# suleka96/siddhi

Hardware: AMD Instinct MI355X
Metric: input events/sec + % HBM peak, partitioned pattern query, 1/2/4/8 MI355X (higher is better)
Workload: dtype f64

## Files before the change

### siddhi_amd/csrc/kernels/stack_dev.h

```cpp
#pragma once
#include "fastpath_dev.h"

namespace sm {
namespace {

constexpr int kKeys = 1024;
#ifndef SM_STACK_KC
#define SM_STACK_KC 5
#endif
constexpr int kC = SM_STACK_KC;
constexpr int kQ = 32;
constexpr int kOB = 1024;
#ifndef SM_ORDER_TB
#define SM_ORDER_TB 13
#endif
constexpr int kTB = SM_ORDER_TB;
constexpr int kOT = 1 << kTB;

enum : uint32_t { SE_OVERFLOW = 1, SE_LOG = 2, SE_NAN = 4, SE_CAND = 8, SE_ORD = 16 };

struct ExactSrc {
  bool exact_codes;
  int vtype, vattr, cwidth;
  const void* vcol;
  const int64_t* ord;
  int64_t obase, n;
  const int64_t* crow;
  int32_t o0;
  uint32_t cs, ce;
  __device__ bool carried(uint32_t o) const { return (int32_t)o < o0; }
  __device__ int64_t row_of(uint32_t o) const {
    if (!ord) return o;
    const int64_t want = (int64_t)o + obase;
    int64_t lo = 0, hi = n - 1;
    while (lo < hi) {
      const int64_t mid = (lo + hi) >> 1;
      if (ord[mid] < want) lo = mid + 1;
      else hi = mid;
    }
    return lo;
  }
  __device__ int64_t carry_row(uint32_t o) const {
    const int64_t want = (int64_t)(int32_t)o + obase;
    uint32_t lo = cs, hi = ce;
    while (lo + 1 < hi) {
      const uint32_t mid = (lo + hi) >> 1;
      if (crow[(int64_t)mid * cwidth + 1] <= want) lo = mid;
      else hi = mid;
    }
    return lo;
  }
  __device__ double fval(uint32_t o) const {
    if (carried(o)) return __longlong_as_double((long long)crow[carry_row(o) * cwidth + 3 + vattr]);
    const int64_t r = row_of(o);
    return vtype == T_FLOAT ? (double)((const float*)vcol)[r] : ((const double*)vcol)[r];
  }
  __device__ int64_t ival(uint32_t o) const {
    if (carried(o)) return crow[carry_row(o) * cwidth + 3 + vattr];
    const int64_t r = row_of(o);
    return vtype == T_INT ? (int64_t)((const int32_t*)vcol)[r] : ((const int64_t*)vcol)[r];
  }
};

#ifndef SM_EXACT_INLINE
#define SM_EXACT_INLINE __noinline__
#endif
template <int OP, bool FP>
__device__ SM_EXACT_INLINE bool c2_exact_v(bool exact_codes, int vtype, int vattr, int cwidth, const void* vcol,
                                        const int64_t* ord, int64_t obase, int64_t n, const int64_t* crow, int32_t o0,
                                        uint32_t cs, uint32_t ce, uint32_t oi, uint32_t oj) {
  const ExactSrc ex{exact_codes, vtype, vattr, cwidth, vcol, ord, obase, n, crow, o0, cs, ce};
  if constexpr (FP) return cmp_fixed<OP>(ex.fval(oj), ex.fval(oi));
  else return cmp_fixed<OP>(ex.ival(oj), ex.ival(oi));
}
template <int OP, bool FP>
__device__ __forceinline__ bool c2_exact(const ExactSrc& ex, uint32_t oi, uint32_t oj) {
  return c2_exact_v<OP, FP>(ex.exact_codes, ex.vtype, ex.vattr, ex.cwidth, ex.vcol, ex.ord, ex.obase, ex.n, ex.crow,
                            ex.o0, ex.cs, ex.ce, oi, oj);
}

template <int OP, bool FP>
__device__ __forceinline__ bool c2_hit(const ExactSrc& ex, uint32_t ci, uint32_t oi, uint32_t cj, uint32_t oj) {
  const bool nan = FP & ((ci == kNanCode) | (cj == kNanCode));
  if (!nan & (ex.exact_codes | (ci != cj))) return cmp_fixed<OP>(cj, ci);
  return c2_exact<OP, FP>(ex, oi, oj);
}

struct Stack {
  uint32_t o[kC], c[kC];
  int32_t t[kC];
  int n;
  int hb, hn;
};

__device__ __forceinline__ void st_pop(Stack& s) {
#pragma unroll
  for (int k = 0; k + 1 < kC; ++k) {
    s.o[k] = s.o[k + 1];
    s.c[k] = s.c[k + 1];
    s.t[k] = s.t[k + 1];
  }
  --s.n;
}

__device__ __forceinline__ void st_refill(Stack& s, const uint4* sp) {
  const uint4 e = sp[(s.hb + s.hn - 1) & (kQ - 1)];
  s.o[0] = e.x;
  s.c[0] = e.y;
  s.t[0] = (int32_t)e.z;
  s.hn -= 1;
  s.n = 1;
}

__device__ __forceinline__ void st_push(Stack& s, uint4* sp, uint32_t o, uint32_t c, int32_t t, int32_t now,
                                        int64_t within, uint32_t* err) {
  if (s.n == kC) {
    if (within >= 0 && now - s.t[kC - 1] > (int32_t)within) {
      s.hn = 0;
      s.n = kC - 1;
    } else {
      if (s.hn == kQ) {
#pragma unroll 1
        while (s.hn > 0 && within >= 0 && now - (int32_t)sp[s.hb & (kQ - 1)].z > (int32_t)within) {
          s.hb = (s.hb + 1) & (kQ - 1);
          --s.hn;
        }
        if (s.hn == kQ) {
          atomicOr(err, SE_OVERFLOW);
          s.hb = (s.hb + 1) & (kQ - 1);
          --s.hn;
        }
      }
      sp[(s.hb + s.hn) & (kQ - 1)] = make_uint4(s.o[kC - 1], s.c[kC - 1], (uint32_t)s.t[kC - 1], 0u);
      ++s.hn;
      s.n = kC - 1;
    }
  }
#pragma unroll
  for (int k = kC - 1; k > 0; --k) {
    s.o[k] = s.o[k - 1];
    s.c[k] = s.c[k - 1];
    s.t[k] = s.t[k - 1];
  }
  s.o[0] = o;
  s.c[0] = c;
  s.t[0] = t;
  ++s.n;
}

template <int NT = kOB>
__device__ __forceinline__ uint32_t block_excl(uint32_t v, uint32_t* lw, uint32_t* tot) {
  const int lane = threadIdx.x & 63, w = threadIdx.x >> 6;
  uint32_t inc = v;
#pragma unroll
  for (int o = 1; o < 64; o <<= 1) {
    const uint32_t u = __shfl_up(inc, o, 64);
    if (lane >= o) inc += u;
  }
  if (lane == 63) lw[w] = inc;
  lds_barrier();
  uint32_t r = inc - v, t = 0;
  for (int q = 0; q < NT / 64; ++q) {
    const uint32_t x = lw[q];
    if (q < w) r += x;
    t += x;
  }
  *tot = t;
  return r;
}

#ifndef SM_STACK_R
#define SM_STACK_R 2
#endif
#ifndef SM_STACK_SS
#define SM_STACK_SS 3072
#endif
constexpr int kR = SM_STACK_R;
constexpr int kSS = SM_STACK_SS;
constexpr int kT4 = kKeys;
constexpr int kW4 = kT4 / 64;
constexpr int kI4 = kSS / kT4;
constexpr int kPool = kSS / 2;
static_assert(kSS % kT4 == 0 && kI4 * 64 <= 255 && kW4 == 16, "u8 per-(key, wave) counts, 16 waves");
static_assert(kSS <= 32768, "arrival positions | c1 fit 16 bits");

struct Slot4 {
  uint2 grp[kSS];
  uint32_t ordt[kSS];
  uint32_t pk[kSS];
  uint2 pool[kPool];
  uint32_t kst[kKeys];
  uint16_t epos[kSS];
  uint8_t jc[kSS];
};
static_assert(sizeof(uint32_t) * kSS + sizeof(uint2) * kPool >= kKeys * kW4, "ranking counts fit pk + pool");

struct Stack4Cold {
  int64_t kmin, ts0, within, obase, n;
  int vtype, vattr, cwidth;
  int32_t o0;
  bool exact_codes;
  const void* vcol;
  const int64_t* ord;
  const uint4* cin;
  const uint32_t* cstart;
  const uint32_t* cend;
  const int64_t* crow;
  int64_t* cand;
  uint32_t* cand_n;
  uint32_t cand_cap;
};

#ifndef SM_EXACT4_INLINE
#define SM_EXACT4_INLINE __noinline__
#endif
struct Stack4Args {
  const uint4* rec;
  const uint32_t* dbase;
  uint32_t n;
  int H;
  int32_t within;
  bool exact_codes;
  uint32_t ntiles;
  const uint32_t* sbase;
  uint64_t* stage;
  uint32_t* mstart;
  uint32_t* mtot;
  uint4* spill;
  uint32_t* err;
  const Stack4Cold* cold;
  unsigned long long* stamps;
};

#ifndef SM_STACK4_SKIP
#define SM_STACK4_SKIP 0
#endif
#ifndef SM_STACK4_STAMPS
#define SM_STACK4_STAMPS 0
#endif
#if SM_STACK4_STAMPS && defined(__HIP_DEVICE_COMPILE__)
#define SM4_CLOCK() __builtin_amdgcn_s_memtime()
#else
#define SM4_CLOCK() 0ull
#endif
#define SM4_PHASE(i)                              \
  do {                                            \
    if (SM_STACK4_STAMPS) {                       \
      const unsigned long long t_ = SM4_CLOCK();  \
      st_acc[i] += t_ - st_last;                  \
      st_last = t_;                               \
    }                                             \
  } while (0)

template <int OP, bool FP>
__device__ SM_EXACT4_INLINE bool c2_exact4(const Stack4Cold* c, uint32_t cs, uint32_t ce, uint32_t oi, uint32_t oj) {
  return c2_exact_v<OP, FP>(c->exact_codes, c->vtype, c->vattr, c->cwidth, c->vcol, c->ord, c->obase, c->n, c->crow,
                            c->o0, cs, ce, oi, oj);
}

__device__ __forceinline__ uint32_t sm4_opaque(uint32_t v) {
#if defined(__HIP_DEVICE_COMPILE__)
  asm volatile("" : "+v"(v));
#endif
  return v;
}

__device__ __forceinline__ void sm4_arrived(uint4 (&pre)[kI4]) {
#if defined(__HIP_DEVICE_COMPILE__)
#pragma unroll
  for (int k = 0; k < kI4; ++k)
    asm volatile("" : "+v"(pre[k].x), "+v"(pre[k].y), "+v"(pre[k].z), "+v"(pre[k].w) : : "memory");
#else
  (void)pre;
#endif
}

#ifndef SM_RANK4_INLINE
#define SM_RANK4_INLINE __forceinline__
#endif
__device__ SM_RANK4_INLINE void rank4(Slot4& S, const uint4 (&pre)[kI4], int sn, uint32_t* lw, bool fp,
                                       uint32_t* err) {
  const int tid = threadIdx.x, lane = tid & 63, w = wave_index();
  uint8_t* cnt = (uint8_t*)S.pk;
  {
    const uint32_t z = sm4_opaque(0u);
    *(uint4*)(cnt + 16 * tid) = make_uint4(z, z, z, z);
  }
  lds_barrier();
  uint32_t hk[kI4], lp[kI4];
  bool nan = false;
#pragma unroll
  for (int k = 0; k < kI4; ++k) {
    const int e = w * 64 * kI4 + k * 64 + lane;
    const bool valid = e < sn;
    nan |= fp && valid && pre[k].z == kNanCode;
    hk[k] = valid ? (pre[k].x & kKeyMask) >> kRB : 0u;
    const uint64_t peers = peer_mask(hk[k], valid);
    uint32_t old = 0;
    if (valid) old = cnt[16 * hk[k] + w];
    wave_lockstep();
    const uint32_t below = lanes_below(peers);
    if (valid && below == 0) cnt[16 * hk[k] + w] = (uint8_t)(old + (uint32_t)__popcll(peers));
    wave_lockstep();
    lp[k] = old + below;
  }
  if (__any(nan) && lane == 0) atomicOr(err, SE_NAN);
  lds_barrier();
  {
    const uint4 c = *(const uint4*)(cnt + 16 * tid);
    const uint32_t ones = 0x01010101u;
    const uint32_t tot = sm_udot4(c.x, ones, 0u) + sm_udot4(c.y, ones, 0u) +
                         sm_udot4(c.z, ones, 0u) + sm_udot4(c.w, ones, 0u);
    uint32_t all;
    const uint32_t st = block_excl<kT4>(tot, lw, &all);
    S.kst[tid] = st | (tot << 16);
  }
  lds_barrier();
#pragma unroll
  for (int k = 0; k < kI4; ++k) {
    const int e = w * 64 * kI4 + k * 64 + lane;
    if (e < sn) {
      const uint4 c = *(const uint4*)(cnt + 16 * hk[k]);
      const uint32_t wb = (uint32_t)w * 8u;
      auto part = [&](uint32_t word, uint32_t lo) {
        const uint32_t nb = wb > lo ? (wb - lo >= 32u ? 32u : wb - lo) : 0u;
        const uint32_t m = nb >= 32u ? 0xffffffffu : ((1u << nb) - 1u);
        return sm_udot4(word & m, 0x01010101u, 0u);
      };
      const uint32_t before = part(c.x, 0) + part(c.y, 32) + part(c.z, 64) + part(c.w, 96);
      const uint32_t pos = (S.kst[hk[k]] & 0xffffu) + before + lp[k];
      S.grp[pos] = make_uint2(pre[k].z, pre[k].w);
      S.epos[pos] = (uint16_t)((uint32_t)e | ((pre[k].x >> 31) << 15));
      S.ordt[e] = pre[k].y;
      if (SM_STACK4_SKIP) S.jc[e] = 0;
    }
  }
  lds_barrier();
}

template <int OP, bool FP>
__global__ void __launch_bounds__(kT4) stack4_kernel(Stack4Args a) {
  __shared__ __attribute__((aligned(16))) Slot4 sl[kR];
  __shared__ uint32_t lw[kW4];
  __shared__ uint32_t s_pool[kR];
  __shared__ uint32_t s_lastj, s_tot;
  const int tid = threadIdx.x, lane = tid & 63;
  const int h = tid;
  const bool has = h < a.H;
  const int32_t within32 = a.within;
  uint4* sp = a.spill + ((int64_t)blockIdx.x * kKeys + h) * kQ;
  unsigned long long st_acc[5] = {0, 0, 0, 0, 0}, st_last = SM4_CLOCK();

  for (int d = blockIdx.x; d < kBins; d += gridDim.x) {
    const uint32_t b0 = a.dbase[d];
    const uint32_t blen = (d + 1 < kBins ? a.dbase[d + 1] : a.n) - b0;
    const uint32_t nsl = (blen + kSS - 1) / kSS;
    const uint4* recb = a.rec + b0;
    uint64_t* stb = a.stage + a.sbase[d];
    uint32_t* mst = a.mstart + (int64_t)d * (a.ntiles + 1);
    const uint32_t kr = ((uint32_t)h << kRB) | (uint32_t)d;
    Stack st;
    st.n = st.hb = st.hn = 0;
    uint32_t cs = 0, ce = 0;
    if (has && a.cold->cin) {
      const Stack4Cold* c4 = a.cold;
      cs = c4->cstart[kr];
      ce = c4->cend[kr];
      for (uint32_t q = cs; q < ce; ++q) {
        const uint4 c = c4->cin[q];
        st_push(st, sp, c.x, c.y, (int32_t)c.z, (int32_t)c.z, within32, a.err);
      }
    }
    int32_t tl = 0;
    bool seen = false;
    uint32_t mrun = 0;
    __syncthreads();
    if (tid == 0) s_lastj = 0xffffffffu;
    if (tid < kR) s_pool[tid] = 0;

    uint4 pre[kI4];
    auto load = [&](uint32_t s) {
#pragma unroll
      for (int k = 0; k < kI4; ++k) {
        const uint32_t p = s * kSS + (uint32_t)wave_index() * 64 * kI4 + k * 64 + lane;
        if (p < blen) {
          typedef unsigned int u32x4 __attribute__((ext_vector_type(4)));
          const u32x4 v = __builtin_nontemporal_load((const u32x4*)recb + p);
          pre[k] = make_uint4(v.x, v.y, v.z, v.w);
        }
      }
    };
    auto slice_n = [&](uint32_t s) { return (int)(blen - s * kSS < (uint32_t)kSS ? blen - s * kSS : (uint32_t)kSS); };
    uint32_t off[kR], cnt[kR];
    SM4_PHASE(4);
    for (uint32_t s = 0; s < (uint32_t)kR; ++s) {
      off[s] = cnt[s] = 0;
      if (s < nsl) {
        load(s);
        rank4(sl[s], pre, slice_n(s), lw, FP, a.err);
        const uint32_t v = sl[s].kst[h];
        off[s] = v & 0xffffu;
        cnt[s] = v >> 16;
      }
    }
    if (kR < nsl) load(kR);

    SM4_PHASE(0);
    for (uint32_t e = 0; e < nsl; ++e) {
      const int q0 = (int)(e % kR);
      while (!SM_STACK4_SKIP && __any(cnt[0] != 0)) {
        int k = kR - 1;
#pragma unroll
        for (int u = kR - 2; u >= 0; --u)
          if (cnt[u]) k = u;
        uint32_t o_ = off[kR - 1], c_ = cnt[kR - 1];
#pragma unroll
        for (int u = kR - 2; u >= 0; --u)
          if (u == k) {
            o_ = off[u];
            c_ = cnt[u];
          }
        if (c_ != 0) {
#pragma unroll
        for (int u = 0; u < kR; ++u)
          if (u == k) {
            off[u] = o_ + 1;
            cnt[u] = c_ - 1;
          }
        const int q = q0 + k >= kR ? q0 + k - kR : q0 + k;
        Slot4& S = sl[q];
        const uint2 g = S.grp[o_];
        const uint32_t ep = S.epos[o_];
        const uint32_t p = ep & 0x7fffu;
        const uint32_t cj = g.x;
        const int32_t jt = (int32_t)g.y;
        tl = jt;
        seen = true;
        uint32_t hit = 0, exp = 0, tie = 0;
#pragma unroll
        for (int u = 0; u < kC; ++u) {
          const bool lv = u < st.n;
          hit |= (lv && cmp_fixed<OP>(cj, st.c[u])) ? (1u << u) : 0u;
          exp |= (lv && within32 >= 0 && jt - st.t[u] > within32) ? (1u << u) : 0u;
          tie |= (lv && !a.exact_codes && st.c[u] == cj) ? (1u << u) : 0u;
        }
        if (tie) {
          const uint32_t oj = S.ordt[p];
#pragma unroll 1
          for (uint32_t m = tie; m; m &= m - 1u) {
            const int u = __builtin_ctz(m);
            uint32_t oi = st.o[0];
#pragma unroll
            for (int v = 1; v < kC; ++v)
              if (v == u) oi = st.o[v];
            if (c2_exact4<OP, FP>(a.cold, cs, ce, oi, oj)) hit |= 1u << u;
            else hit &= ~(1u << u);
          }
        }
        const uint32_t ok = hit & ~exp;
        uint32_t npop = (uint32_t)__builtin_ctz(~ok);
        if (npop > (uint32_t)st.n) npop = st.n;
        const bool stop_expired = npop < (uint32_t)st.n && ((exp >> npop) & 1u);
        const bool cont = !stop_expired && npop == (uint32_t)st.n && st.hn > 0;
        if (npop) S.pk[p] = st.o[0];
        if (npop > 1) {
          const uint32_t base = atomicAdd(&s_pool[q], npop - 1u);
          if (base + npop - 1u > (uint32_t)kPool) atomicOr(a.err, SE_LOG);
#pragma unroll
          for (int u = 1; u < kC; ++u)
            if ((uint32_t)u < npop && base + u - 1u < (uint32_t)kPool)
              S.pool[base + u - 1u] = make_uint2(st.o[u], p | ((uint32_t)u << 16));
        }
#pragma unroll
        for (int b = 1; b < kC; b <<= 1)
          if (npop & b) {
#pragma unroll
            for (int u = 0; u < kC; ++u)
              if (u + b < kC) {
                st.o[u] = st.o[u + b];
                st.c[u] = st.c[u + b];
                st.t[u] = st.t[u + b];
              }
          }
        st.n -= (int)npop;
        if (stop_expired) {
          st.n = 0;
          st.hn = 0;
        } else if (cont) {
#pragma unroll 1
          for (;;) {
            st_refill(st, sp);
            if (within32 >= 0 && jt - st.t[0] > within32) {
              st.n = 0;
              st.hn = 0;
              break;
            }
            const bool hh = (a.exact_codes | (st.c[0] != cj)) ? cmp_fixed<OP>(cj, st.c[0])
                                                               : c2_exact4<OP, FP>(a.cold, cs, ce, st.o[0], S.ordt[p]);
            if (!hh) break;
            if (npop == 0) {
              S.pk[p] = st.o[0];
            } else {
              const uint32_t b1 = atomicAdd(&s_pool[q], 1u);
              if (b1 < (uint32_t)kPool) S.pool[b1] = make_uint2(st.o[0], p | (npop << 16));
              else atomicOr(a.err, SE_LOG);
            }
            ++npop;
            st_pop(st);
            if (st.hn == 0) break;
          }
        }
        S.jc[p] = (uint8_t)npop;
        if (ep >> 15) st_push(st, sp, S.ordt[p], cj, jt, jt, within32, a.err);
        }
      }
      SM4_PHASE(1);
      lds_barrier();
      SM4_PHASE(2);
      sm4_arrived(pre);

      {
        Slot4& S = sl[q0];
        const int sn = slice_n(e);
        uint32_t v[kI4], sum = 0;
#pragma unroll
        for (int k = 0; k < kI4; ++k) {
          const int p = tid * kI4 + k;
          v[k] = p < sn ? S.jc[p] : 0u;
          sum += v[k];
        }
        uint32_t tot;
        uint32_t r = block_excl<kT4>(sum, lw, &tot);
        const uint32_t jprev = s_lastj;
#pragma unroll
        for (int k = 0; k < kI4; ++k) {
          const int p = tid * kI4 + k;
          if (p < sn) {
            S.epos[p] = (uint16_t)r;
            const uint32_t j = S.ordt[p];
            const uint32_t jp = p == 0 ? jprev : S.ordt[p - 1];
            const uint32_t t0 = jp == 0xffffffffu ? 0u : (jp >> kTB) + 1u;
            for (uint32_t t = t0; t <= (j >> kTB); ++t) mst[t] = mrun + r;
            if (v[k]) stb[mrun + r + v[k] - 1u] = ((uint64_t)j << 32) | S.pk[p];
          }
          r += v[k];
        }
        if (tid == 0) s_tot = tot;
        lds_barrier();
        const uint32_t np = s_pool[q0] < (uint32_t)kPool ? s_pool[q0] : (uint32_t)kPool;
        for (uint32_t k = sm4_opaque((uint32_t)tid); k < np; k += kT4) {
          const uint2 pe = S.pool[k];
          const uint32_t p = pe.y & 0xffffu, kk = pe.y >> 16;
#ifdef SM_EMU_DEBUG
          if (kk >= S.jc[p] || p >= (uint32_t)sn) {
            printf("bad pool entry k=%u/%u p=%u kk=%u jc=%u epos=%u sn=%d e=%u q0=%d d=%d\n", k, np, p, kk, S.jc[p], S.epos[p], sn, e, q0, d);
            continue;
          }
#endif
          stb[mrun + S.epos[p] + S.jc[p] - 1u - kk] = ((uint64_t)S.ordt[p] << 32) | pe.x;
        }
        mrun += s_tot;
        lds_barrier();
        if (tid == 0) {
          s_lastj = S.ordt[sn - 1];
          s_pool[q0] = 0;
        }
      }
      SM4_PHASE(3);
      off[0] = off[1];
      cnt[0] = cnt[1];
#pragma unroll
      for (int u = 1; u + 1 < kR; ++u) {
        off[u] = off[u + 1];
        cnt[u] = cnt[u + 1];
      }
      off[kR - 1] = cnt[kR - 1] = 0;
      if (e + kR < nsl) {
        rank4(sl[q0], pre, slice_n(e + kR), lw, FP, a.err);
        const uint32_t vv = sl[q0].kst[h];
        off[kR - 1] = vv & 0xffffu;
        cnt[kR - 1] = vv >> 16;
        if (e + kR + 1 < nsl) load(e + kR + 1);
      }
      SM4_PHASE(0);
    }
    __syncthreads();
    {
      const uint32_t jl = s_lastj;
      const uint32_t t0 = jl == 0xffffffffu ? 0u : (jl >> kTB) + 1u;
      for (uint32_t t = t0 + tid; t <= (uint32_t)a.ntiles; t += kT4) mst[t] = mrun;
      if (tid == 0) a.mtot[d] = mrun;
    }

    auto pending = [&](int32_t t) { return !seen || within32 < 0 || (int64_t)tl - t <= within32; };
    uint32_t keep = 0;
    if (has) {
#pragma unroll
      for (int k = 0; k < kC; ++k)
        if (k < st.n && pending(st.t[k])) ++keep;
      for (int k = 0; k < st.hn; ++k)
        if (pending((int32_t)sp[(st.hb + k) & (kQ - 1)].z)) ++keep;
    }
    uint32_t inc = keep;
#pragma unroll
    for (int o = 1; o < 64; o <<= 1) {
      const uint32_t u = __shfl_up(inc, o, 64);
      if (lane >= o) inc += u;
    }
    uint32_t base = 0;
    const Stack4Cold* c4 = a.cold;
    if (lane == 63 && inc) base = atomicAdd(c4->cand_n, inc);
    base = __shfl(base, 63, 64) + inc - keep;
    if (keep) {
      const ExactSrc ex{c4->exact_codes, c4->vtype, c4->vattr, c4->cwidth, c4->vcol, c4->ord, c4->obase, c4->n,
                        c4->crow, c4->o0, cs, ce};
      const int64_t key = c4->kmin + (int64_t)kr;
      auto put = [&](uint32_t o, int32_t t) {
        if (!pending(t)) return;
        if (base < c4->cand_cap) {
          int64_t* c = c4->cand + 4 * (int64_t)base;
          c[0] = key;
          c[1] = (int64_t)(int32_t)o + c4->obase;
          c[2] = (int64_t)t + c4->ts0;
          c[3] = ex.carried(o) ? -(int64_t)ex.carry_row(o) - 1 : ex.row_of(o);
        } else {
          atomicOr(a.err, SE_CAND);
        }
        ++base;
      };
      for (int k = 0; k < st.hn; ++k) {
        const uint4 c = sp[(st.hb + k) & (kQ - 1)];
        put(c.x, (int32_t)c.z);
      }
#pragma unroll
      for (int k = kC - 1; k >= 0; --k)
        if (k < st.n) put(st.o[k], st.t[k]);
    }
  }
  SM4_PHASE(4);
  if (SM_STACK4_STAMPS && a.stamps && lane == 0)
    for (int i = 0; i < 5; ++i) atomicAdd(&a.stamps[i], st_acc[i]);
}

}
}
```

Measured before the change: 25.78 billion.

## Add branchless flat fast path for per-event stack update with padded slots

Pads unused stack slots with sentinel codes and times, so hit and expiry counts become simple unmasked comparisons over all slots. Each event's pop, push, spill, clear and refill is then done as a predicated barrel shift instead of divergent branching. The old general path stays for tie cases or a full spill ring. The goal is less wave divergence and a shorter dependency chain in the per-event loop, at the cost of more instructions per event and extra register pressure. It also adds a host-emulation invariant check.

```diff
diff --git a/siddhi_amd/csrc/kernels/stack_dev.h b/siddhi_amd/csrc/kernels/stack_dev.h
--- a/siddhi_amd/csrc/kernels/stack_dev.h
+++ b/siddhi_amd/csrc/kernels/stack_dev.h
@@ -1,5 +1,9 @@
 #pragma once
 #include "fastpath_dev.h"
+#ifdef SM_HOST_EMU
+#include <cstdio>
+#include <cstdlib>
+#endif
 
 namespace sm {
 namespace {
@@ -148,6 +152,21 @@
   ++s.n;
 }
 
+constexpr int32_t kPadT = 1 << 30;
+template <int OP>
+__device__ __forceinline__ constexpr uint32_t pad_code() {
+  return (OP == CMP_LT || OP == CMP_LE) ? 0u : 0xffffffffu;
+}
+template <int OP>
+__device__ __forceinline__ void st_pad(Stack& s) {
+#pragma unroll
+  for (int k = 0; k < kC; ++k)
+    if (k >= s.n) {
+      s.c[k] = pad_code<OP>();
+      s.t[k] = kPadT;
+    }
+}
+
 template <int NT = kOB>
 __device__ __forceinline__ uint32_t block_excl(uint32_t v, uint32_t* lw, uint32_t* tot) {
   const int lane = threadIdx.x & 63, w = threadIdx.x >> 6;
@@ -235,6 +254,9 @@
 #ifndef SM_STACK4_SKIP
 #define SM_STACK4_SKIP 0
 #endif
+#ifndef SM_STACK4_FLAT
+#define SM_STACK4_FLAT 1
+#endif
 #ifndef SM_STACK4_STAMPS
 #define SM_STACK4_STAMPS 0
 #endif
@@ -338,6 +360,24 @@
   lds_barrier();
 }
 
+#ifdef SM_HOST_EMU
+template <int OP>
+inline void sm4_check_step(const Stack& st, uint32_t cj, int32_t jt, int32_t weff, int nhit, int nexp) {
+  bool ok = st.n >= 0 && st.n <= kC && nexp <= st.n;
+  for (int u = 0; u < kC; ++u) {
+    if (u >= st.n) ok = ok && st.c[u] == pad_code<OP>() && st.t[u] == kPadT;
+    ok = ok && cmp_fixed<OP>(cj, st.c[u]) == (u < nhit);
+    ok = ok && (jt - st.t[u] > weff) == (u >= st.n - nexp && u < st.n);
+    if (u > 0 && u < st.n) ok = ok && st.t[u] <= st.t[u - 1];
+  }
+  if (!ok) {
+    fprintf(stderr, "stack4 event step: invariant broken (n %d, nhit %d, nexp %d, code %u, time %d)\n", st.n, nhit,
+            nexp, cj, jt);
+    abort();
+  }
+}
+#endif
+
 template <int OP, bool FP>
 __global__ void __launch_bounds__(kT4) stack4_kernel(Stack4Args a) {
   __shared__ __attribute__((aligned(16))) Slot4 sl[kR];
@@ -348,6 +388,7 @@
   const int h = tid;
   const bool has = h < a.H;
   const int32_t within32 = a.within;
+  const int32_t weff = within32 < 0 ? INT32_MAX : within32;
   uint4* sp = a.spill + ((int64_t)blockIdx.x * kKeys + h) * kQ;
   unsigned long long st_acc[5] = {0, 0, 0, 0, 0}, st_last = SM4_CLOCK();
 
@@ -361,6 +402,8 @@
     const uint32_t kr = ((uint32_t)h << kRB) | (uint32_t)d;
     Stack st;
     st.n = st.hb = st.hn = 0;
+#pragma unroll
+    for (int k = 0; k < kC; ++k) st.o[k] = 0;
     uint32_t cs = 0, ce = 0;
     if (has && a.cold->cin) {
       const Stack4Cold* c4 = a.cold;
@@ -371,6 +414,7 @@
         st_push(st, sp, c.x, c.y, (int32_t)c.z, (int32_t)c.z, within32, a.err);
       }
     }
+    st_pad<OP>(st);
     int32_t tl = 0;
     bool seen = false;
     uint32_t mrun = 0;
@@ -408,34 +452,155 @@
     SM4_PHASE(0);
     for (uint32_t e = 0; e < nsl; ++e) {
       const int q0 = (int)(e % kR);
-      while (!SM_STACK4_SKIP && __any(cnt[0] != 0)) {
+      if (!SM_STACK4_SKIP && __any(cnt[0] != 0)) do {
         int k = kR - 1;
-#pragma unroll
-        for (int u = kR - 2; u >= 0; --u)
-          if (cnt[u]) k = u;
         uint32_t o_ = off[kR - 1], c_ = cnt[kR - 1];
-#pragma unroll
-        for (int u = kR - 2; u >= 0; --u)
-          if (u == k) {
-            o_ = off[u];
-            c_ = cnt[u];
-          }
-        if (c_ != 0) {
-#pragma unroll
-        for (int u = 0; u < kR; ++u)
-          if (u == k) {
-            off[u] = o_ + 1;
-            cnt[u] = c_ - 1;
-          }
+        if constexpr (kR == 2) {
+          k = cnt[0] != 0 ? 0 : 1;
+          o_ = k ? off[1] : off[0];
+          c_ = k ? cnt[1] : cnt[0];
+        } else {
+#pragma unroll
+          for (int u = kR - 2; u >= 0; --u)
+            if (cnt[u]) k = u;
+#pragma unroll
+          for (int u = kR - 2; u >= 0; --u)
+            if (u == k) {
+              o_ = off[u];
+              c_ = cnt[u];
+            }
+        }
+        const bool act = c_ != 0;
+        if constexpr (kR == 2) {
+          const uint32_t a0 = k == 0 ? 1u : 0u, a1 = ((k != 0) & act) ? 1u : 0u;
+          off[0] += a0;
+          cnt[0] -= a0;
+          off[1] += a1;
+          cnt[1] -= a1;
+        } else {
+#pragma unroll
+          for (int u = 0; u < kR; ++u)
+            if ((u == k) & act) {
+              off[u] = o_ + 1;
+              cnt[u] = c_ - 1;
+            }
+        }
         const int q = q0 + k >= kR ? q0 + k - kR : q0 + k;
         Slot4& S = sl[q];
-        const uint2 g = S.grp[o_];
-        const uint32_t ep = S.epos[o_];
-        const uint32_t p = ep & 0x7fffu;
+        const uint32_t oa = act ? o_ : 0u;
+        const uint2 g = S.grp[oa];
+        const uint32_t ep = S.epos[oa];
+        const uint32_t p = act ? ep & 0x7fffu : 0u;
+        const uint32_t oj = S.ordt[p];
+        const bool push = (ep >> 15) != 0;
         const uint32_t cj = g.x;
         const int32_t jt = (int32_t)g.y;
-        tl = jt;
-        seen = true;
+        tl = act ? jt : tl;
+        seen |= act;
+        int nhit = 0, nexp = 0;
+        bool anytie = false;
+#pragma unroll
+        for (int u = 0; u < kC; ++u) {
+          nhit += cmp_fixed<OP>(cj, st.c[u]) ? 1 : 0;
+          nexp += jt - st.t[u] > weff ? 1 : 0;
+          anytie |= st.c[u] == cj;
+        }
+        const int nl = st.n - nexp;
+        const int nmin = nhit < nl ? nhit : nl;
+        const bool clr = (nexp != 0) & (nl <= nhit);
+        const int nrem = clr ? 0 : st.n - nmin;
+        const bool full = push & (nrem == kC);
+        const bool spill = full & (nexp == 0), refill = (nexp == 0) & (nhit >= st.n) & (st.hn > 0);
+        const bool general = !SM_STACK4_FLAT | (anytie & !a.exact_codes) | (spill & (st.hn == kQ));
+        const bool flat = act & !general;
+#ifdef SM_HOST_EMU
+        if (flat) sm4_check_step<OP>(st, cj, jt, weff, nhit, nexp);
+#endif
+        const uint32_t np = flat ? (uint32_t)nmin : 0u;
+        const bool clear = flat & clr, pushf = flat & push, ring0 = flat & (clr | (full & !spill));
+        if (flat & spill) {
+          sp[(st.hb + st.hn) & (kQ - 1)] = make_uint4(st.o[kC - 1], st.c[kC - 1], (uint32_t)st.t[kC - 1], 0u);
+          ++st.hn;
+        }
+        if (np) S.pk[p] = st.o[0];
+        if (np > 1) {
+          const uint32_t base = atomicAdd(&s_pool[q], np - 1u);
+          if (base + np - 1u > (uint32_t)kPool) atomicOr(a.err, SE_LOG);
+#pragma unroll
+          for (int u = 1; u < kC; ++u)
+            if ((uint32_t)u < np && base + u - 1u < (uint32_t)kPool)
+              S.pool[base + u - 1u] = make_uint2(st.o[u], p | ((uint32_t)u << 16));
+        }
+        if (flat) S.jc[p] = (uint8_t)np;
+        {
+          constexpr int top = kC >= 8 ? 8 : kC >= 4 ? 4 : 2;
+          static_assert(kC < 2 * top, "the shift's bits cover kC");
+          const uint32_t sh = clear ? (uint32_t)kC : np;
+#pragma unroll
+          for (int b = top; b >= 1; b >>= 1) {
+            const bool on = (sh & (uint32_t)b) != 0;
+#pragma unroll
+            for (int u = 0; u < kC; ++u) {
+              if (u + b < kC) {
+                st.o[u] = on ? st.o[u + b] : st.o[u];
+                st.c[u] = on ? st.c[u + b] : st.c[u];
+                st.t[u] = on ? st.t[u + b] : st.t[u];
+              } else {
+                st.c[u] = on ? pad_code<OP>() : st.c[u];
+                st.t[u] = on ? kPadT : st.t[u];
+              }
+            }
+          }
+#pragma unroll
+          for (int u = kC - 1; u > 0; --u) {
+            st.o[u] = pushf ? st.o[u - 1] : st.o[u];
+            st.c[u] = pushf ? st.c[u - 1] : st.c[u];
+            st.t[u] = pushf ? st.t[u - 1] : st.t[u];
+          }
+          st.o[0] = pushf ? oj : st.o[0];
+          st.c[0] = pushf ? cj : st.c[0];
+          st.t[0] = pushf ? jt : st.t[0];
+          st.n = flat ? nrem + ((push & !full) ? 1 : 0) : st.n;
+          st.hn = ring0 ? 0 : st.hn;
+        }
+        if (__builtin_expect(flat & refill, 0)) {
+          uint32_t npop = np;
+#pragma unroll 1
+          for (;;) {
+            const uint4 e = sp[(st.hb + st.hn - 1) & (kQ - 1)];
+            if (jt - (int32_t)e.z > weff) {
+              st.hn = 0;
+              break;
+            }
+            const bool hh = (a.exact_codes | (e.y != cj)) ? cmp_fixed<OP>(cj, e.y)
+                                                          : c2_exact4<OP, FP>(a.cold, cs, ce, e.x, oj);
+            st.hn -= 1;
+            if (!hh) {
+              if (push) {
+                st.o[1] = e.x;
+                st.c[1] = e.y;
+                st.t[1] = (int32_t)e.z;
+              } else {
+                st.o[0] = e.x;
+                st.c[0] = e.y;
+                st.t[0] = (int32_t)e.z;
+              }
+              st.n += 1;
+              break;
+            }
+            if (npop == 0) {
+              S.pk[p] = e.x;
+            } else {
+              const uint32_t b1 = atomicAdd(&s_pool[q], 1u);
+              if (b1 < (uint32_t)kPool) S.pool[b1] = make_uint2(e.x, p | (npop << 16));
+              else atomicOr(a.err, SE_LOG);
+            }
+            ++npop;
+            if (st.hn == 0) break;
+          }
+          S.jc[p] = (uint8_t)npop;
+        }
+        if (__builtin_expect(act & general, 0)) {
         uint32_t hit = 0, exp = 0, tie = 0;
 #pragma unroll
         for (int u = 0; u < kC; ++u) {
@@ -445,7 +610,6 @@
           tie |= (lv && !a.exact_codes && st.c[u] == cj) ? (1u << u) : 0u;
         }
         if (tie) {
-          const uint32_t oj = S.ordt[p];
 #pragma unroll 1
           for (uint32_t m = tie; m; m &= m - 1u) {
             const int u = __builtin_ctz(m);
@@ -496,7 +660,7 @@
               break;
             }
             const bool hh = (a.exact_codes | (st.c[0] != cj)) ? cmp_fixed<OP>(cj, st.c[0])
-                                                               : c2_exact4<OP, FP>(a.cold, cs, ce, st.o[0], S.ordt[p]);
+                                                               : c2_exact4<OP, FP>(a.cold, cs, ce, st.o[0], oj);
             if (!hh) break;
             if (npop == 0) {
               S.pk[p] = st.o[0];
@@ -511,9 +675,10 @@
           }
         }
         S.jc[p] = (uint8_t)npop;
-        if (ep >> 15) st_push(st, sp, S.ordt[p], cj, jt, jt, within32, a.err);
-        }
-      }
+        if (push) st_push(st, sp, oj, cj, jt, jt, within32, a.err);
+        st_pad<OP>(st);
+        }
+      } while (__any(cnt[0] != 0));
       SM4_PHASE(1);
       lds_barrier();
       SM4_PHASE(2);
```

After: 26.70 billion (median of 6 runs). +3.5%, better.
